# simonmeister/UnFlow

Hardware: NVIDIA H100
Metric: frame-pairs/s at 384x1280 FlowNetC (higher is better)
Workload: dtype f32

## Files before the change

### unflow_b200/csrc/tc_common.cuh

```cuda
#pragma once
#include <cuda.h>

#include "common.cuh"

namespace unflow {
namespace tc {

constexpr int BM = 128;
constexpr int BK = 32;
constexpr int CHUNK = 8;
constexpr int A_BYTES = BM * BK * 4;
extern long long *g_dbg;
extern int g_chunk;

__device__ __forceinline__ unsigned s32(const void *p) { return (unsigned)__cvta_generic_to_shared(p); }

__device__ __forceinline__ void mbar_init(unsigned bar, int count) {
  asm volatile("mbarrier.init.shared::cta.b64 [%0], %1;" ::"r"(bar), "r"(count));
}
__device__ __forceinline__ void mbar_arrive(unsigned bar) {
  asm volatile("mbarrier.arrive.shared::cta.b64 _, [%0];" ::"r"(bar) : "memory");
}
__device__ __forceinline__ void mbar_expect_tx(unsigned bar, unsigned bytes) {
  asm volatile("mbarrier.arrive.expect_tx.shared::cta.b64 _, [%0], %1;" ::"r"(bar), "r"(bytes) : "memory");
}
__device__ __forceinline__ void mbar_wait(unsigned bar, unsigned parity) {
  unsigned done;
  do {
    asm volatile(
        "{\n .reg .pred p;\n mbarrier.try_wait.parity.shared::cta.b64 p, [%1], %2;\n"
        " selp.u32 %0, 1, 0, p;\n}\n"
        : "=r"(done) : "r"(bar), "r"(parity) : "memory");
  } while (!done);
}
__device__ __forceinline__ bool elect_one() {
  unsigned pred = 0;
  asm volatile("{\n .reg .pred p;\n elect.sync _|p, 0xFFFFFFFF;\n selp.u32 %0, 1, 0, p;\n}\n" : "=r"(pred));
  return pred != 0;
}
__device__ __forceinline__ void tma_4d(unsigned dst, const CUtensorMap *map, unsigned bar, int c0, int c1,
                                       int c2, int c3) {
  asm volatile(
      "cp.async.bulk.tensor.4d.shared::cluster.global.tile.mbarrier::complete_tx::bytes"
      " [%0], [%1, {%3, %4, %5, %6}], [%2];"
      ::"r"(dst), "l"(map), "r"(bar), "r"(c0), "r"(c1), "r"(c2), "r"(c3) : "memory");
}
__device__ __forceinline__ void tma_3d(unsigned dst, const CUtensorMap *map, unsigned bar, int c0, int c1,
                                       int c2) {
  asm volatile(
      "cp.async.bulk.tensor.3d.shared::cluster.global.tile.mbarrier::complete_tx::bytes"
      " [%0], [%1, {%3, %4, %5}], [%2];"
      ::"r"(dst), "l"(map), "r"(bar), "r"(c0), "r"(c1), "r"(c2) : "memory");
}
__device__ __forceinline__ void fence_proxy_async() {
  asm volatile("fence.proxy.async.shared::cta;" ::: "memory");
}
__device__ __forceinline__ void named_bar_sync(int id, int count) {
  asm volatile("bar.sync %0, %1;" ::"r"(id), "r"(count) : "memory");
}

__device__ __forceinline__ float tf32_rna(float x) {
  unsigned u;
  asm("cvt.rna.tf32.f32 %0, %1;" : "=r"(u) : "f"(x));
  return __uint_as_float(u);
}
__device__ __forceinline__ float tf32_rna_fast(float x) {
  return __uint_as_float((__float_as_uint(x) + 0x1000u) & 0xFFFFE000u);
}
__device__ __forceinline__ float4 tf32_hi4(float4 v) {
  return make_float4(tf32_rna_fast(v.x), tf32_rna_fast(v.y), tf32_rna_fast(v.z), tf32_rna_fast(v.w));
}
__device__ __forceinline__ float4 sub4(float4 a, float4 b) { return make_float4(a.x - b.x, a.y - b.y, a.z - b.z, a.w - b.w); }

__device__ __forceinline__ void red_add_f32(float *addr, float v) {
  asm volatile("red.global.add.f32 [%0], %1;" ::"l"(addr), "f"(v) : "memory");
}

__device__ __forceinline__ unsigned long long wgmma_desc_k128(unsigned saddr) {
  return (unsigned long long)((saddr >> 4) & 0x3FFFu) | (1ull << 16) | (64ull << 32) | (1ull << 62);
}
__device__ __forceinline__ unsigned sw128_offset(int r, int k) {
  return (unsigned)(r * 128 + ((((k >> 2) ^ (r & 7)) & 7) << 4) + ((k & 3) << 2));
}
__device__ __forceinline__ void wgmma_fence() { asm volatile("wgmma.fence.sync.aligned;" ::: "memory"); }
__device__ __forceinline__ void wgmma_commit() { asm volatile("wgmma.commit_group.sync.aligned;" ::: "memory"); }
template <int N>
__device__ __forceinline__ void wgmma_wait() { asm volatile("wgmma.wait_group.sync.aligned %0;" ::"n"(N) : "memory"); }
template <int R>
__device__ __forceinline__ void fence_regs(float (&d)[R]) {
#pragma unroll
  for (int i = 0; i < R; ++i) asm volatile("" : "+f"(d[i])::"memory");
}
template <int N> struct Wgmma;
template <> struct Wgmma<32> {
  static __device__ __forceinline__ void mma(float (&d)[16], unsigned long long da, unsigned long long db, int scale_d) {
    asm volatile(
        "{\n .reg .pred p;\n setp.ne.b32 p, %18, 0;\n"
        " wgmma.mma_async.sync.aligned.m64n32k8.f32.tf32.tf32 {%0, %1, %2, %3, %4, %5, %6, %7, %8, %9, %10, %11, %12, %13, %14, %15}, %16, %17, p, 1, 1;\n}\n"
        : "+f"(d[0]), "+f"(d[1]), "+f"(d[2]), "+f"(d[3]), "+f"(d[4]), "+f"(d[5]), "+f"(d[6]), "+f"(d[7]), "+f"(d[8]), "+f"(d[9]), "+f"(d[10]), "+f"(d[11]), "+f"(d[12]), "+f"(d[13]), "+f"(d[14]), "+f"(d[15])
        : "l"(da), "l"(db), "r"(scale_d));
  }
};
template <> struct Wgmma<64> {
  static __device__ __forceinline__ void mma(float (&d)[32], unsigned long long da, unsigned long long db, int scale_d) {
    asm volatile(
        "{\n .reg .pred p;\n setp.ne.b32 p, %34, 0;\n"
        " wgmma.mma_async.sync.aligned.m64n64k8.f32.tf32.tf32 {%0, %1, %2, %3, %4, %5, %6, %7, %8, %9, %10, %11, %12, %13, %14, %15, %16, %17, %18, %19, %20, %21, %22, %23, %24, %25, %26, %27, %28, %29, %30, %31}, %32, %33, p, 1, 1;\n}\n"
        : "+f"(d[0]), "+f"(d[1]), "+f"(d[2]), "+f"(d[3]), "+f"(d[4]), "+f"(d[5]), "+f"(d[6]), "+f"(d[7]), "+f"(d[8]), "+f"(d[9]), "+f"(d[10]), "+f"(d[11]), "+f"(d[12]), "+f"(d[13]), "+f"(d[14]), "+f"(d[15]), "+f"(d[16]), "+f"(d[17]), "+f"(d[18]), "+f"(d[19]), "+f"(d[20]), "+f"(d[21]), "+f"(d[22]), "+f"(d[23]), "+f"(d[24]), "+f"(d[25]), "+f"(d[26]), "+f"(d[27]), "+f"(d[28]), "+f"(d[29]), "+f"(d[30]), "+f"(d[31])
        : "l"(da), "l"(db), "r"(scale_d));
  }
};
template <> struct Wgmma<128> {
  static __device__ __forceinline__ void mma(float (&d)[64], unsigned long long da, unsigned long long db, int scale_d) {
    asm volatile(
        "{\n .reg .pred p;\n setp.ne.b32 p, %66, 0;\n"
        " wgmma.mma_async.sync.aligned.m64n128k8.f32.tf32.tf32 {%0, %1, %2, %3, %4, %5, %6, %7, %8, %9, %10, %11, %12, %13, %14, %15, %16, %17, %18, %19, %20, %21, %22, %23, %24, %25, %26, %27, %28, %29, %30, %31, %32, %33, %34, %35, %36, %37, %38, %39, %40, %41, %42, %43, %44, %45, %46, %47, %48, %49, %50, %51, %52, %53, %54, %55, %56, %57, %58, %59, %60, %61, %62, %63}, %64, %65, p, 1, 1;\n}\n"
        : "+f"(d[0]), "+f"(d[1]), "+f"(d[2]), "+f"(d[3]), "+f"(d[4]), "+f"(d[5]), "+f"(d[6]), "+f"(d[7]), "+f"(d[8]), "+f"(d[9]), "+f"(d[10]), "+f"(d[11]), "+f"(d[12]), "+f"(d[13]), "+f"(d[14]), "+f"(d[15]), "+f"(d[16]), "+f"(d[17]), "+f"(d[18]), "+f"(d[19]), "+f"(d[20]), "+f"(d[21]), "+f"(d[22]), "+f"(d[23]), "+f"(d[24]), "+f"(d[25]), "+f"(d[26]), "+f"(d[27]), "+f"(d[28]), "+f"(d[29]), "+f"(d[30]), "+f"(d[31]), "+f"(d[32]), "+f"(d[33]), "+f"(d[34]), "+f"(d[35]), "+f"(d[36]), "+f"(d[37]), "+f"(d[38]), "+f"(d[39]), "+f"(d[40]), "+f"(d[41]), "+f"(d[42]), "+f"(d[43]), "+f"(d[44]), "+f"(d[45]), "+f"(d[46]), "+f"(d[47]), "+f"(d[48]), "+f"(d[49]), "+f"(d[50]), "+f"(d[51]), "+f"(d[52]), "+f"(d[53]), "+f"(d[54]), "+f"(d[55]), "+f"(d[56]), "+f"(d[57]), "+f"(d[58]), "+f"(d[59]), "+f"(d[60]), "+f"(d[61]), "+f"(d[62]), "+f"(d[63])
        : "l"(da), "l"(db), "r"(scale_d));
  }
};

typedef CUresult (*EncodeTiledFn)(CUtensorMap *, CUtensorMapDataType, cuuint32_t, void *, const cuuint64_t *,
                                  const cuuint64_t *, const cuuint32_t *, const cuuint32_t *,
                                  CUtensorMapInterleave, CUtensorMapSwizzle, CUtensorMapL2promotion,
                                  CUtensorMapFloatOOBfill);
inline EncodeTiledFn encode_fn() {
  static EncodeTiledFn fn = nullptr;
  static bool tried = false;
  if (!tried) {
    tried = true;
    void *ptr = nullptr;
    cudaDriverEntryPointQueryResult q;
    if (cudaGetDriverEntryPoint("cuTensorMapEncodeTiled", &ptr, cudaEnableDefault, &q) == cudaSuccess &&
        q == cudaDriverEntryPointSuccess)
      fn = (EncodeTiledFn)ptr;
  }
  return fn;
}
inline int encode(CUtensorMap *m, const float *basep, int rank, const cuuint64_t *dims,
                  const cuuint64_t *strides_bytes, const cuuint32_t *box, const cuuint32_t *estr,
                  CUtensorMapSwizzle swizzle = CU_TENSOR_MAP_SWIZZLE_128B) {
  if (bind_primary_context()) return UNFLOW_ECUDA;
  EncodeTiledFn fn = encode_fn();
  if (!fn) { set_error("cuTensorMapEncodeTiled entry point not available"); return UNFLOW_ECUDA; }
  CUresult r = fn(m, CU_TENSOR_MAP_DATA_TYPE_FLOAT32, (cuuint32_t)rank, (void *)basep, dims, strides_bytes, box,
                  estr, CU_TENSOR_MAP_INTERLEAVE_NONE, swizzle,
                  CU_TENSOR_MAP_L2_PROMOTION_L2_256B, CU_TENSOR_MAP_FLOAT_OOB_FILL_NONE);
  if (r != CUDA_SUCCESS) { set_error("cuTensorMapEncodeTiled failed (%d)", (int)r); return UNFLOW_ECUDA; }
  return UNFLOW_OK;
}

}
}
```

### unflow_b200/csrc/tc_conv.cu

```cuda
#include <algorithm>

#include "tc_common.cuh"

namespace unflow {
namespace tc {

constexpr int MAX_TAPS = 64;
constexpr int NTHREADS = 384;

struct Tap {
  short dx, dy;
  int widx;
  int widx2;
};

struct ConvParams {
  int N, Hit, Wit;
  int TW, TH, TN;
  int tiles_x, tiles_y, tiles_n, n_blocks, n_classes;
  int s_in_x, s_in_y, s_out;
  int Cin, Cout, kblocks;
  float *out;
  long long out_pitch;
  int Hout, Wout;
  const float *bias;
  float slope;
  int act, accumulate;
  int chunk;
  long long *dbg;
  int pair_px;
  int ksplit;
  int class_start[5];
  short class_px[4], class_py[4];
  Tap taps[MAX_TAPS];
};

template <int BN>
struct Cfg {
  static constexpr int B_BYTES = BN * BK * 4;
  static constexpr int STAGE_BYTES = 2 * A_BYTES + 2 * B_BYTES;
  static constexpr int B_OFF = 2 * A_BYTES;
  static constexpr int STAGES = (200 * 1024 / STAGE_BYTES) < 8 ? (200 * 1024 / STAGE_BYTES) : 8;
  static constexpr int SMEM_BYTES = STAGES * STAGE_BYTES + 1024  + 256 ;
  static_assert(STAGES >= 2, "at least two stages");
};

struct TileCoord {
  int cls, n0, iy0, ix0, nb;
};
__device__ __forceinline__ TileCoord decode_tile(const ConvParams &p, int tile) {
  TileCoord t;
  t.nb = tile % p.n_blocks; tile /= p.n_blocks;
  t.cls = tile % p.n_classes; tile /= p.n_classes;
  t.ix0 = (tile % p.tiles_x) * p.TW; tile /= p.tiles_x;
  t.iy0 = (tile % p.tiles_y) * p.TH; tile /= p.tiles_y;
  t.n0 = tile * p.TN;
  return t;
}

struct Work {
  TileCoord t;
  int it0, iters;
};
__device__ __forceinline__ Work decode_work(const ConvParams &p, int w) {
  Work k;
  const int tile = w / p.ksplit, ks = w - tile * p.ksplit;
  k.t = decode_tile(p, tile);
  const int total = (p.class_start[k.t.cls + 1] - p.class_start[k.t.cls]) * p.kblocks;
  const int per = (total + p.ksplit - 1) / p.ksplit;
  k.it0 = ks * per;
  k.iters = total - k.it0 < per ? total - k.it0 : per;
  if (k.iters < 0) k.iters = 0;
  return k;
}

template <int BN>
__global__ void __launch_bounds__(NTHREADS, 1)
tc_conv_kernel(const __grid_constant__ CUtensorMap mapA, const __grid_constant__ CUtensorMap mapBhi,
               const __grid_constant__ CUtensorMap mapBlo, const __grid_constant__ ConvParams p) {
  using C = Cfg<BN>;
  constexpr int R = BN / 2;
  extern __shared__ unsigned char smem_raw[];
  const unsigned base = (s32(smem_raw) + 1023u) & ~1023u;
  unsigned char *gbase = smem_raw + (base - s32(smem_raw));
  const unsigned bars = base + C::STAGES * C::STAGE_BYTES;
  auto full = [&](int s) { return bars + 8u * s; };
  auto empty = [&](int s) { return bars + 8u * (C::STAGES + s); };

  const int warp = __shfl_sync(0xffffffffu, threadIdx.x >> 5, 0), lane = threadIdx.x & 31;
  const int m_tiles = p.tiles_n * p.tiles_y * p.tiles_x;
  const int total_items = p.n_classes * m_tiles * p.n_blocks * p.ksplit;

  if (threadIdx.x == 0) {
    for (int s = 0; s < C::STAGES; ++s) {
      mbar_init(full(s), 1);
      mbar_init(empty(s), 8);
    }
    asm volatile("fence.mbarrier_init.release.cluster;" ::: "memory");
    asm volatile("prefetch.tensormap [%0];" ::"l"(&mapA) : "memory");
    asm volatile("prefetch.tensormap [%0];" ::"l"(&mapBhi) : "memory");
    asm volatile("prefetch.tensormap [%0];" ::"l"(&mapBlo) : "memory");
  }
  __syncthreads();

  if (warp == 0) {
    int s = 0;
    unsigned ph = 0;
    long long t_wait = 0, t_all = clock64();
    const unsigned a_box_bytes = (unsigned)(p.TW * p.TH * p.TN) * BK * 4u;
    for (int item = blockIdx.x; item < total_items; item += gridDim.x) {
      const Work wk = decode_work(p, item);
      const TileCoord t = wk.t;
      const int x0 = p.s_in_x * t.ix0, y0 = p.s_in_y * t.iy0;
      int ti = p.class_start[t.cls] + wk.it0 / p.kblocks, kc = wk.it0 % p.kblocks;
      for (int it = 0; it < wk.iters; ++it) {
        const Tap tap = p.taps[ti];
        { const long long t0 = clock64(); mbar_wait(empty(s), ph ^ 1u); t_wait += clock64() - t0; }
        const unsigned st = base + s * C::STAGE_BYTES;
        if (elect_one()) {
          mbar_expect_tx(full(s), a_box_bytes + 2u * C::B_BYTES);
          tma_4d(st, &mapA, full(s), kc * BK, x0 + tap.dx, y0 + tap.dy, t.n0);
          if (p.pair_px) {
            const int w0 = tap.widx < 0 ? (1 << 20) : tap.widx, w1 = tap.widx2 < 0 ? (1 << 20) : tap.widx2;
            tma_3d(st + C::B_OFF, &mapBhi, full(s), kc * BK, 0, w0);
            tma_3d(st + C::B_OFF + C::B_BYTES / 2, &mapBhi, full(s), kc * BK, 0, w1);
            tma_3d(st + C::B_OFF + C::B_BYTES, &mapBlo, full(s), kc * BK, 0, w0);
            tma_3d(st + C::B_OFF + C::B_BYTES + C::B_BYTES / 2, &mapBlo, full(s), kc * BK, 0, w1);
          } else {
            tma_3d(st + C::B_OFF, &mapBhi, full(s), kc * BK, t.nb * BN, tap.widx);
            tma_3d(st + C::B_OFF + C::B_BYTES, &mapBlo, full(s), kc * BK, t.nb * BN, tap.widx);
          }
        }
        __syncwarp();
        if (++s == C::STAGES) { s = 0; ph ^= 1u; }
        if (++kc == p.kblocks) { kc = 0; ++ti; }
      }
    }
    if (p.dbg && blockIdx.x == 0 && lane == 0) { p.dbg[0] = t_wait; p.dbg[1] = clock64() - t_all; }
  } else if (warp >= 4) {
    const int cw = (warp >> 2) - 1;
    const int ct = threadIdx.x - 128 * (cw + 1);
    const int row0 = 64 * cw + 16 * (ct >> 5) + (lane >> 2);
    const int col0 = 2 * (lane & 3);
    const int per_img = p.TW * p.TH;
    int s = 0;
    unsigned ph = 0;
    long long t_wait = 0, t_all = clock64();
    float sum[R], acc[R];
    for (int item = blockIdx.x; item < total_items; item += gridDim.x) {
      const Work wk = decode_work(p, item);
      const TileCoord t = wk.t;
      const int iters = wk.iters;
#pragma unroll
      for (int c = 0; c < R; ++c) sum[c] = 0.f;
      for (int c0 = 0; c0 < iters; c0 += p.chunk) {
        const int c1 = c0 + p.chunk < iters ? c0 + p.chunk : iters;
        int pending = -1;
        for (int it = c0; it < c1; ++it) {
          { const long long t0 = clock64(); mbar_wait(full(s), ph); t_wait += clock64() - t0; }
          {
            float4 *a = reinterpret_cast<float4 *>(gbase + s * C::STAGE_BYTES + cw * (A_BYTES / 2));
            float4 *l = reinterpret_cast<float4 *>(gbase + s * C::STAGE_BYTES + A_BYTES + cw * (A_BYTES / 2));
#pragma unroll
            for (int j = 0; j < A_BYTES / 2 / 16 / 128; ++j) {
              const int i = ct + 128 * j;
              const float4 v = a[i], h = tf32_hi4(v);
              a[i] = h;
              l[i] = sub4(v, h);
            }
          }
          fence_proxy_async();
          named_bar_sync(1 + cw, 128);
          const unsigned st = base + s * C::STAGE_BYTES;
          const unsigned long long a_hi = wgmma_desc_k128(st + cw * (A_BYTES / 2));
          const unsigned long long a_lo = wgmma_desc_k128(st + A_BYTES + cw * (A_BYTES / 2));
          const unsigned long long b_hi = wgmma_desc_k128(st + C::B_OFF), b_lo = wgmma_desc_k128(st + C::B_OFF + C::B_BYTES);
          fence_regs(acc);
          wgmma_fence();
#pragma unroll
          for (int k = 0; k < BK / 8; ++k) {
            const unsigned long long adv = (unsigned long long)(2 * k);
            Wgmma<BN>::mma(acc, a_lo + adv, b_hi + adv, (it - c0 | k) != 0);
            Wgmma<BN>::mma(acc, a_hi + adv, b_lo + adv, 1);
            Wgmma<BN>::mma(acc, a_hi + adv, b_hi + adv, 1);
          }
          wgmma_commit();
          wgmma_wait<1>();
          fence_regs(acc);
          __syncwarp();
          if (pending >= 0 && lane == 0) mbar_arrive(empty(pending));
          pending = s;
          if (++s == C::STAGES) { s = 0; ph ^= 1u; }
        }
        wgmma_wait<0>();
        fence_regs(acc);
        __syncwarp();
        if (lane == 0) mbar_arrive(empty(pending));
#pragma unroll
        for (int c = 0; c < R; ++c) sum[c] += acc[c];
      }
#pragma unroll
      for (int h = 0; h < 2; ++h) {
        const int row = row0 + 8 * h;
        const int tn = row / per_img, rem = row - tn * per_img;
        const int ty = rem / p.TW, tx = rem - ty * p.TW;
        const int n = t.n0 + tn, iy = t.iy0 + ty, ix = t.ix0 + tx;
        if (!(tn < p.TN && n < p.N && iy < p.Hit && ix < p.Wit)) continue;
        const int oy = p.s_out * iy + p.class_py[t.cls];
        float *const orow = p.out + ((long long)n * p.Hout + oy) * p.Wout * p.out_pitch;
#pragma unroll
        for (int j = 0; j < BN / 8; ++j) {
          const int col = 8 * j + col0;
          const int half = p.pair_px && col >= BN / 2 ? 1 : 0;
          const int c = p.pair_px ? col - half * (BN / 2) : t.nb * BN + col;
          const int ox = p.s_out * ix + (p.pair_px ? half : p.class_px[t.cls]);
          if (c >= p.Cout) continue;
          float *dst = orow + (long long)ox * p.out_pitch + c;
          float v0 = sum[4 * j + 2 * h], v1 = sum[4 * j + 2 * h + 1];
          const bool two = c + 1 < p.Cout;
          if (p.ksplit > 1) {
            if (iters > 0) {
              red_add_f32(dst, v0);
              if (two) red_add_f32(dst + 1, v1);
            }
            continue;
          }
          if (p.bias) {
            v0 += __ldg(p.bias + c);
            if (two) v1 += __ldg(p.bias + c + 1);
          }
          if (p.act) {
            v0 = v0 > 0.f ? v0 : p.slope * v0;
            v1 = v1 > 0.f ? v1 : p.slope * v1;
          }
          if (two) {
            float2 *o = reinterpret_cast<float2 *>(dst);
            if (p.accumulate) { const float2 old = *o; v0 += old.x; v1 += old.y; }
            *o = make_float2(v0, v1);
          } else {
            *dst = p.accumulate ? *dst + v0 : v0;
          }
        }
      }
    }
    if (p.dbg && blockIdx.x == 0 && threadIdx.x == 128) { p.dbg[2] = t_wait; p.dbg[3] = clock64() - t_all; }
  }
}

__global__ void __launch_bounds__(256)
wsplit_kernel(const float *__restrict__ w, float *__restrict__ hi, float *__restrict__ lo, int taps, int R,
              int C, int Cp, long long s_t, long long s_r, long long s_c, int r_fast) {
  __shared__ float tile[32][33];
  const int t = blockIdx.z;
  const int r0 = blockIdx.y * 32, c0 = blockIdx.x * 32;
  const int tx = threadIdx.x & 31, ty = threadIdx.x >> 5;
  for (int k = ty; k < 32; k += 8) {
    const int r = r0 + (r_fast ? tx : k), c = c0 + (r_fast ? k : tx);
    float v = 0.f;
    if (r < R && c < C) v = w[t * s_t + r * s_r + c * s_c];
    if (r_fast) tile[tx][k] = v; else tile[k][tx] = v;
  }
  __syncthreads();
  for (int k = ty; k < 32; k += 8) {
    const int r = r0 + k, c = c0 + tx;
    if (r < R && c < Cp) {
      const float v = tile[k][tx];
      const float h = tf32_rna(v);
      const long long o = ((long long)t * R + r) * Cp + c;
      hi[o] = h;
      lo[o] = v - h;
    }
  }
}

static int floordiv(int a, int b) { return (a >= 0) ? a / b : -((-a + b - 1) / b); }

int g_chunk = CHUNK;
int g_pair_px = 1;
int g_ksplit = 1;
long long *g_dbg = nullptr;

template <int BN>
static int launch(const CUtensorMap &mA, const CUtensorMap &mBh, const CUtensorMap &mBl, const ConvParams &p,
                  cudaStream_t stream) {
  using C = Cfg<BN>;
  static bool attr_set = false;
  if (!attr_set) {
    cudaError_t e = cudaFuncSetAttribute(tc_conv_kernel<BN>, cudaFuncAttributeMaxDynamicSharedMemorySize, C::SMEM_BYTES);
    if (e != cudaSuccess) { set_error("tc_conv: cannot opt in to %d bytes of shared memory: %s", C::SMEM_BYTES, cudaGetErrorString(e)); return UNFLOW_ECUDA; }
    attr_set = true;
  }
  const long long total = (long long)p.n_classes * p.tiles_n * p.tiles_y * p.tiles_x * p.n_blocks * p.ksplit;
  const int grid = total < kNumSMs ? (int)total : kNumSMs;
  tc_conv_kernel<BN><<<grid, NTHREADS, C::SMEM_BYTES, stream>>>(mA, mBh, mBl, p);
  count_launch();
  return check_launch("tc_conv_kernel");
}

inline int choose_ksplit(const ConvParams &p) {
  if (!g_ksplit) return 1;
  const long long items = (long long)p.n_classes * p.tiles_n * p.tiles_y * p.tiles_x * p.n_blocks;
  if (2 * items > kNumSMs) return 1;
  int min_iters = 1 << 30;
  for (int c = 0; c < p.n_classes; ++c) min_iters = std::min(min_iters, (p.class_start[c + 1] - p.class_start[c]) * p.kblocks);
  const long long ks = std::min<long long>(std::min<long long>(kNumSMs / items, 4), std::max(1, min_iters / (4 * p.chunk)));
  return ks < 1 ? 1 : (int)ks;
}

static int launch_bn(int BN, const CUtensorMap &mA, const float *w_hi, const float *w_lo, const cuuint64_t *wdims,
                     const cuuint64_t *wstrides, const ConvParams &p, cudaStream_t stream) {
  CUtensorMap mBh, mBl;
  cuuint32_t box[3] = {(cuuint32_t)BK, (cuuint32_t)(p.pair_px ? BN / 2 : BN), 1};
  cuuint32_t estr[3] = {1, 1, 1};
  int rc = encode(&mBh, w_hi, 3, wdims, wstrides, box, estr);
  if (rc) return rc;
  rc = encode(&mBl, w_lo, 3, wdims, wstrides, box, estr);
  if (rc) return rc;
  if (BN == 128) return launch<128>(mA, mBh, mBl, p, stream);
  if (BN == 64) return launch<64>(mA, mBh, mBl, p, stream);
  return launch<32>(mA, mBh, mBl, p, stream);
}

}
int set_tc_chunk(int v) { if (v < 1 || v > 64) return 0; tc::g_chunk = v; return 1; }
int set_tc_ksplit(int v) { if (v != 0 && v != 1) return 0; tc::g_ksplit = v; return 1; }
int set_tc_pair_px(int v) { if (v != 0 && v != 1) return 0; tc::g_pair_px = v; return 1; }
}

using namespace unflow;

extern "C" int unflow_bias_lrelu(float *y, const float *bias, long long pixels, int C, float slope, void *stream);

extern "C" int unflow_tc_wsplit(const float *w, float *w_hi, float *w_lo, int taps, int R, int C, long long s_t,
                                long long s_r, long long s_c, void *stream) {
  UNFLOW_REQUIRE(w && w_hi && w_lo && taps > 0 && R > 0 && C > 0, "tc_wsplit: bad arguments");
  UNFLOW_REQUIRE(taps <= 65535 && (R + 31) / 32 <= 65535, "tc_wsplit: too many taps / rows");
  const int Cp = (C + 3) / 4 * 4;
  dim3 grid((Cp + 31) / 32, (R + 31) / 32, taps);
  tc::wsplit_kernel<<<grid, 256, 0, (cudaStream_t)stream>>>(w, w_hi, w_lo, taps, R, C, Cp, s_t, s_r, s_c,
                                                           (s_r == 1 && s_c != 1) ? 1 : 0);
  count_launch();
  return check_launch("tc_wsplit_kernel");
}

static int make_plan(tc::ConvParams &p, int &BN, int N, int Hin, int Win, int Cin, int Hout, int Wout, int Cout,
                     int mode, int stride, int kh, int kw, int pad_t, int pad_l) {
  UNFLOW_REQUIRE(N > 0 && Hin > 0 && Win > 0 && Cin > 0 && Hout > 0 && Wout > 0 && Cout > 0, "tc_conv: bad extents");
  UNFLOW_REQUIRE(mode == 0 || mode == 1, "tc_conv: mode must be 0 (conv) or 1 (transposed)");
  UNFLOW_REQUIRE(stride == 1 || stride == 2, "tc_conv: stride must be 1 or 2");
  UNFLOW_REQUIRE(kh > 0 && kw > 0 && kh * kw <= tc::MAX_TAPS, "tc_conv: at most %d taps", tc::MAX_TAPS);
  p.N = N; p.Cin = Cin; p.Cout = Cout; p.kblocks = (Cin + tc::BK - 1) / tc::BK; p.chunk = tc::g_chunk; p.dbg = tc::g_dbg; p.ksplit = 1;
  p.Hout = Hout; p.Wout = Wout;
  int nt = 0;
  if (mode == 0) {
    p.n_classes = 1; p.s_in_x = p.s_in_y = stride; p.s_out = 1; p.Hit = Hout; p.Wit = Wout;
    p.class_px[0] = p.class_py[0] = 0;
    p.class_start[0] = 0;
    for (int ky = 0; ky < kh; ++ky)
      for (int kx = 0; kx < kw; ++kx) p.taps[nt++] = tc::Tap{(short)(kx - pad_l), (short)(ky - pad_t), ky * kw + kx};
    p.class_start[1] = nt;
  } else {
    UNFLOW_REQUIRE(Hout % stride == 0 && Wout % stride == 0, "tc_conv: transposed output extents must be multiples of the stride");
    p.n_classes = stride * stride; p.s_in_x = p.s_in_y = 1; p.s_out = stride; p.Hit = Hout / stride; p.Wit = Wout / stride;
    int c = 0;
    for (int py = 0; py < stride; ++py)
      for (int px = 0; px < stride; ++px, ++c) {
        p.class_px[c] = (short)px; p.class_py[c] = (short)py;
        p.class_start[c] = nt;
        for (int ky = 0; ky < kh; ++ky) {
          if (((py + pad_t - ky) % stride + stride) % stride) continue;
          for (int kx = 0; kx < kw; ++kx) {
            if (((px + pad_l - kx) % stride + stride) % stride) continue;
            UNFLOW_REQUIRE(nt < tc::MAX_TAPS, "tc_conv: too many taps");
            p.taps[nt++] = tc::Tap{(short)tc::floordiv(px + pad_l - kx, stride),
                                   (short)tc::floordiv(py + pad_t - ky, stride), ky * kw + kx};
          }
        }
      }
    p.class_start[p.n_classes] = nt;
    for (int c2 = 0; c2 < p.n_classes; ++c2)
      UNFLOW_REQUIRE(p.class_start[c2 + 1] > p.class_start[c2], "tc_conv: an output parity class has no taps");
  }
  long long best = -1;
  for (int TW = 1; TW <= p.Wit && TW <= 128; ++TW)
    for (int TH = 1; TH <= p.Hit && TW * TH <= 128; ++TH) {
      int TN = 128 / (TW * TH);
      if (TN > N) TN = N;
      const long long tiles = (long long)((p.Wit + TW - 1) / TW) * ((p.Hit + TH - 1) / TH) * ((N + TN - 1) / TN);
      if (best < 0 || tiles < best || (tiles == best && TW > p.TW)) {
        best = tiles; p.TW = TW; p.TH = TH; p.TN = TN;
      }
    }
  p.tiles_x = (p.Wit + p.TW - 1) / p.TW; p.tiles_y = (p.Hit + p.TH - 1) / p.TH; p.tiles_n = (N + p.TN - 1) / p.TN;
  BN = Cout > 64 ? 128 : (Cout > 32 ? 64 : 32);
  p.n_blocks = (Cout + BN - 1) / BN;
  const long long total = (long long)p.n_classes * p.tiles_n * p.tiles_y * p.tiles_x * p.n_blocks;
  UNFLOW_REQUIRE(total < (1ll << 30), "tc_conv: too many tiles");
  return UNFLOW_OK;
// ... 135 lines not shown
```

### unflow_b200/csrc/tc_wgrad.cu

```cuda
#include "tc_common.cuh"

namespace unflow {
namespace tcw {

using namespace unflow::tc;

constexpr int NTHREADS = 384;
constexpr int KP = 32;

struct WgradParams {
  int N, Hp, Wp;
  int TW, TH, TN;
  int tiles_x, tiles_y, tiles_n;
  int n_ptiles, kc, n_chunks;
  int R, C;
  int cgroups, vgroups;
  int r_blocks, c_blocks, taps, kw;
  int chunk;
  long long *dbg;
  int stride, stride_x, pad_t, pad_l;
  float *dw;
  long long pitch_r, pitch_t;
};

constexpr int SMEM_LIMIT = 232448;

template <int BN>
struct Cfg {
  static constexpr int G_BYTES = BN * KP * 4;
  static constexpr int A_HI = 0;
  static constexpr int A_LO = A_HI + A_BYTES;
  static constexpr int B_HI = A_LO + A_BYTES;
  static constexpr int B_LO = B_HI + G_BYTES;
  static constexpr int SPLIT_BYTES = B_LO + G_BYTES;
  static constexpr int SPLIT_STAGES = 2;
  static constexpr int G_RAW = A_BYTES;
  static constexpr int RAW_BYTES = A_BYTES + G_BYTES;
  static constexpr int RAW0 = SPLIT_STAGES * SPLIT_BYTES;
  static constexpr int FIXED = RAW0 + 1024  + 256 ;
  static constexpr int RAW_STAGES = (SMEM_LIMIT - FIXED) / RAW_BYTES < 8 ? (SMEM_LIMIT - FIXED) / RAW_BYTES : 8;
  static constexpr int SMEM_BYTES = FIXED + RAW_STAGES * RAW_BYTES;
  static_assert(RAW_STAGES >= 3, "TMA at least two K blocks ahead of the split");
  static_assert(SMEM_BYTES <= SMEM_LIMIT, "over the shared memory of a block");
  static_assert(8 * (2 * RAW_STAGES + SPLIT_STAGES) <= 256, "barriers");
};

struct Item {
  int chunk, rb, cb;
};
__device__ __forceinline__ Item decode_item(const WgradParams &p, int it) {
  Item w;
  w.cb = it % p.c_blocks; it /= p.c_blocks;
  w.rb = it % p.r_blocks; it /= p.r_blocks;
  w.chunk = it;
  return w;
}
__device__ __forceinline__ int chunk_len(const WgradParams &p, int chunk) {
  const int k0 = chunk * p.kc;
  return (k0 + p.kc <= p.n_ptiles) ? p.kc : p.n_ptiles - k0;
}

template <int ROWS>
__device__ __forceinline__ void split_transpose(const float *raw, unsigned char *hi, unsigned char *lo, int row0, int ct) {
#pragma unroll
  for (int j = 0; j < ROWS * 8 / 128; ++j) {
    const int i = ct + 128 * j;
    const int r = row0 + i % ROWS, c = i / ROWS;
    const float *src = raw + (r >> 5) * 1024 + (4 * c) * 32 + (r & 31);
    const float4 v = make_float4(src[0], src[32], src[64], src[96]), h = tf32_hi4(v);
    const unsigned o = sw128_offset(r, 4 * c);
    *reinterpret_cast<float4 *>(hi + o) = h;
    *reinterpret_cast<float4 *>(lo + o) = sub4(v, h);
  }
}

template <int BN>
__global__ void __launch_bounds__(NTHREADS, 1)
tc_wgrad_kernel(const __grid_constant__ CUtensorMap mapP, const __grid_constant__ CUtensorMap mapG,
                const __grid_constant__ WgradParams p) {
  using C = Cfg<BN>;
  constexpr int R = BN / 2;
  constexpr int GROUPS = BN / 32;
  extern __shared__ unsigned char smem_raw[];
  const unsigned base = (s32(smem_raw) + 1023u) & ~1023u;
  unsigned char *gbase = smem_raw + (base - s32(smem_raw));
  const unsigned bars = base + C::RAW0 + C::RAW_STAGES * C::RAW_BYTES;
  auto raw_full = [&](int s) { return bars + 8u * s; };
  auto raw_empty = [&](int s) { return bars + 8u * (C::RAW_STAGES + s); };
  auto split_empty = [&](int s) { return bars + 8u * (2 * C::RAW_STAGES + s); };

  const int warp = __shfl_sync(0xffffffffu, threadIdx.x >> 5, 0), lane = threadIdx.x & 31;
  const int total_items = p.n_chunks * p.r_blocks * p.c_blocks;

  if (threadIdx.x == 0) {
    for (int s = 0; s < C::RAW_STAGES; ++s) {
      mbar_init(raw_full(s), 1);
      mbar_init(raw_empty(s), 8);
    }
    for (int s = 0; s < C::SPLIT_STAGES; ++s) mbar_init(split_empty(s), 8);
    asm volatile("fence.mbarrier_init.release.cluster;" ::: "memory");
    asm volatile("prefetch.tensormap [%0];" ::"l"(&mapP) : "memory");
    asm volatile("prefetch.tensormap [%0];" ::"l"(&mapG) : "memory");
  }
  __syncthreads();

  if (warp == 0) {
    int s = 0;
    unsigned ph = 0;
    long long t_wait = 0, t_all = clock64();
    for (int item = blockIdx.x; item < total_items; item += gridDim.x) {
      const Item w = decode_item(p, item);
      int gch[GROUPS], gdx[GROUPS], gdy[GROUPS];
#pragma unroll
      for (int j = 0; j < GROUPS; ++j) {
        const int v = w.cb * GROUPS + j;
        if (v < p.vgroups) {
          const int tap = v / p.cgroups, ky = tap / p.kw;
          gch[j] = (v - tap * p.cgroups) * 32; gdy[j] = ky - p.pad_t; gdx[j] = tap - ky * p.kw - p.pad_l;
        } else {
          gch[j] = p.cgroups * 32; gdx[j] = gdy[j] = 0;
        }
      }
      const int k0 = w.chunk * p.kc, klen = chunk_len(p, w.chunk);
      for (int kb = k0; kb < k0 + klen; ++kb) {
        int q = kb;
        const int px = (q % p.tiles_x) * p.TW; q /= p.tiles_x;
        const int py = (q % p.tiles_y) * p.TH; q /= p.tiles_y;
        const int pn = q * p.TN;
        { const long long t0 = clock64(); mbar_wait(raw_empty(s), ph ^ 1u); t_wait += clock64() - t0; }
        const unsigned st = base + C::RAW0 + s * C::RAW_BYTES;
        if (elect_one()) {
          mbar_expect_tx(raw_full(s), (unsigned)C::RAW_BYTES);
#pragma unroll
          for (int j = 0; j < BM / 32; ++j)
            tma_4d(st + j * 4096, &mapP, raw_full(s), w.rb * BM + 32 * j, px, py, pn);
#pragma unroll
          for (int j = 0; j < GROUPS; ++j)
            tma_4d(st + C::G_RAW + j * 4096, &mapG, raw_full(s), gch[j], p.stride_x * px + gdx[j],
                   p.stride * py + gdy[j], pn);
        }
        __syncwarp();
        if (++s == C::RAW_STAGES) { s = 0; ph ^= 1u; }
      }
    }
    if (p.dbg && blockIdx.x == 0 && lane == 0) { p.dbg[0] = t_wait; p.dbg[1] = clock64() - t_all; }
  } else if (warp >= 4) {
    const int cw = (warp >> 2) - 1;
    const int ct = threadIdx.x - 128 * (cw + 1);
    const int row0 = 64 * cw + 16 * (ct >> 5) + (lane >> 2);
    const int col0 = 2 * (lane & 3);
    unsigned n = 0;
    unsigned t_wait = 0, t_split = 0;
    const unsigned t_all = (unsigned)clock();
    auto split = [&](bool rows) {
      const unsigned rs = n % C::RAW_STAGES, rph = (n / C::RAW_STAGES) & 1u;
      const unsigned ss = n % C::SPLIT_STAGES, sph = (n / C::SPLIT_STAGES) & 1u;
      { const unsigned t0 = (unsigned)clock(); mbar_wait(raw_full(rs), rph); t_wait += (unsigned)clock() - t0; }
      { const unsigned t0 = (unsigned)clock(); mbar_wait(split_empty(ss), sph ^ 1u); t_split += (unsigned)clock() - t0; }
      const float *raw = reinterpret_cast<const float *>(gbase + C::RAW0 + rs * C::RAW_BYTES);
      unsigned char *sp = gbase + ss * C::SPLIT_BYTES;
      if (rows) split_transpose<64>(raw, sp + C::A_HI, sp + C::A_LO, 64 * cw, ct);
      split_transpose<BN / 2>(raw + C::G_RAW / 4, sp + C::B_HI, sp + C::B_LO, cw * (BN / 2), ct);
      __syncwarp();
      if (lane == 0) mbar_arrive(raw_empty(rs));
      fence_proxy_async();
      named_bar_sync(1, 256);
    };
    float sum[R], acc[R];
    for (int item = blockIdx.x; item < total_items; item += gridDim.x) {
      const Item w = decode_item(p, item);
      const int iters = chunk_len(p, w.chunk);
      if (w.rb * BM + 64 * cw >= p.R) {
        for (int it = 0; it < iters; ++it) {
          split(false);
          if (lane == 0) mbar_arrive(split_empty(n % C::SPLIT_STAGES));
          ++n;
        }
        continue;
// ... 198 lines not shown
```

Before: 136.2.

## Split A operand into tf32 hi/lo in registers and feed register-sourced WGMMA

The conv kernel no longer rewrites the A tile in shared memory as separate hi/lo tf32 halves, which needed a proxy fence and a named barrier per K block. Each consumer now loads its A fragment from the swizzled stage, splits it into hi/lo registers, and issues register-A WGMMAs. Commits are per k-step with a double-buffered fragment set so the split overlaps the in-flight MMAs. Because the lo copy of A is gone, each stage is smaller, so more stages fit under a raised shared-memory limit. setmaxnreg moves registers from producer warps to consumer warps, at the cost of more shared loads per thread and tighter wgmma_wait ordering.

```diff
diff --git a/unflow_b200/csrc/tc_common.cuh b/unflow_b200/csrc/tc_common.cuh
--- a/unflow_b200/csrc/tc_common.cuh
+++ b/unflow_b200/csrc/tc_common.cuh
@@ -10,6 +10,7 @@
 constexpr int BK = 32;
 constexpr int CHUNK = 8;
 constexpr int A_BYTES = BM * BK * 4;
+constexpr int SMEM_LIMIT = 232448;
 extern long long *g_dbg;
 extern int g_chunk;
 
@@ -55,6 +56,10 @@
 __device__ __forceinline__ void fence_proxy_async() {
   asm volatile("fence.proxy.async.shared::cta;" ::: "memory");
 }
+template <int N>
+__device__ __forceinline__ void setmaxnreg_dec() { asm volatile("setmaxnreg.dec.sync.aligned.u32 %0;" ::"n"(N)); }
+template <int N>
+__device__ __forceinline__ void setmaxnreg_inc() { asm volatile("setmaxnreg.inc.sync.aligned.u32 %0;" ::"n"(N)); }
 __device__ __forceinline__ void named_bar_sync(int id, int count) {
   asm volatile("bar.sync %0, %1;" ::"r"(id), "r"(count) : "memory");
 }
@@ -100,6 +105,13 @@
         : "+f"(d[0]), "+f"(d[1]), "+f"(d[2]), "+f"(d[3]), "+f"(d[4]), "+f"(d[5]), "+f"(d[6]), "+f"(d[7]), "+f"(d[8]), "+f"(d[9]), "+f"(d[10]), "+f"(d[11]), "+f"(d[12]), "+f"(d[13]), "+f"(d[14]), "+f"(d[15])
         : "l"(da), "l"(db), "r"(scale_d));
   }
+  static __device__ __forceinline__ void mma_rs(float (&d)[16], const unsigned (&a)[4], unsigned long long db, int scale_d) {
+    asm volatile(
+        "{\n .reg .pred p;\n setp.ne.b32 p, %21, 0;\n"
+        " wgmma.mma_async.sync.aligned.m64n32k8.f32.tf32.tf32 {%0, %1, %2, %3, %4, %5, %6, %7, %8, %9, %10, %11, %12, %13, %14, %15}, {%16, %17, %18, %19}, %20, p, 1, 1;\n}\n"
+        : "+f"(d[0]), "+f"(d[1]), "+f"(d[2]), "+f"(d[3]), "+f"(d[4]), "+f"(d[5]), "+f"(d[6]), "+f"(d[7]), "+f"(d[8]), "+f"(d[9]), "+f"(d[10]), "+f"(d[11]), "+f"(d[12]), "+f"(d[13]), "+f"(d[14]), "+f"(d[15])
+        : "r"(a[0]), "r"(a[1]), "r"(a[2]), "r"(a[3]), "l"(db), "r"(scale_d));
+  }
 };
 template <> struct Wgmma<64> {
   static __device__ __forceinline__ void mma(float (&d)[32], unsigned long long da, unsigned long long db, int scale_d) {
@@ -109,6 +121,13 @@
         : "+f"(d[0]), "+f"(d[1]), "+f"(d[2]), "+f"(d[3]), "+f"(d[4]), "+f"(d[5]), "+f"(d[6]), "+f"(d[7]), "+f"(d[8]), "+f"(d[9]), "+f"(d[10]), "+f"(d[11]), "+f"(d[12]), "+f"(d[13]), "+f"(d[14]), "+f"(d[15]), "+f"(d[16]), "+f"(d[17]), "+f"(d[18]), "+f"(d[19]), "+f"(d[20]), "+f"(d[21]), "+f"(d[22]), "+f"(d[23]), "+f"(d[24]), "+f"(d[25]), "+f"(d[26]), "+f"(d[27]), "+f"(d[28]), "+f"(d[29]), "+f"(d[30]), "+f"(d[31])
         : "l"(da), "l"(db), "r"(scale_d));
   }
+  static __device__ __forceinline__ void mma_rs(float (&d)[32], const unsigned (&a)[4], unsigned long long db, int scale_d) {
+    asm volatile(
+        "{\n .reg .pred p;\n setp.ne.b32 p, %37, 0;\n"
+        " wgmma.mma_async.sync.aligned.m64n64k8.f32.tf32.tf32 {%0, %1, %2, %3, %4, %5, %6, %7, %8, %9, %10, %11, %12, %13, %14, %15, %16, %17, %18, %19, %20, %21, %22, %23, %24, %25, %26, %27, %28, %29, %30, %31}, {%32, %33, %34, %35}, %36, p, 1, 1;\n}\n"
+        : "+f"(d[0]), "+f"(d[1]), "+f"(d[2]), "+f"(d[3]), "+f"(d[4]), "+f"(d[5]), "+f"(d[6]), "+f"(d[7]), "+f"(d[8]), "+f"(d[9]), "+f"(d[10]), "+f"(d[11]), "+f"(d[12]), "+f"(d[13]), "+f"(d[14]), "+f"(d[15]), "+f"(d[16]), "+f"(d[17]), "+f"(d[18]), "+f"(d[19]), "+f"(d[20]), "+f"(d[21]), "+f"(d[22]), "+f"(d[23]), "+f"(d[24]), "+f"(d[25]), "+f"(d[26]), "+f"(d[27]), "+f"(d[28]), "+f"(d[29]), "+f"(d[30]), "+f"(d[31])
+        : "r"(a[0]), "r"(a[1]), "r"(a[2]), "r"(a[3]), "l"(db), "r"(scale_d));
+  }
 };
 template <> struct Wgmma<128> {
   static __device__ __forceinline__ void mma(float (&d)[64], unsigned long long da, unsigned long long db, int scale_d) {
@@ -117,6 +136,13 @@
         " wgmma.mma_async.sync.aligned.m64n128k8.f32.tf32.tf32 {%0, %1, %2, %3, %4, %5, %6, %7, %8, %9, %10, %11, %12, %13, %14, %15, %16, %17, %18, %19, %20, %21, %22, %23, %24, %25, %26, %27, %28, %29, %30, %31, %32, %33, %34, %35, %36, %37, %38, %39, %40, %41, %42, %43, %44, %45, %46, %47, %48, %49, %50, %51, %52, %53, %54, %55, %56, %57, %58, %59, %60, %61, %62, %63}, %64, %65, p, 1, 1;\n}\n"
         : "+f"(d[0]), "+f"(d[1]), "+f"(d[2]), "+f"(d[3]), "+f"(d[4]), "+f"(d[5]), "+f"(d[6]), "+f"(d[7]), "+f"(d[8]), "+f"(d[9]), "+f"(d[10]), "+f"(d[11]), "+f"(d[12]), "+f"(d[13]), "+f"(d[14]), "+f"(d[15]), "+f"(d[16]), "+f"(d[17]), "+f"(d[18]), "+f"(d[19]), "+f"(d[20]), "+f"(d[21]), "+f"(d[22]), "+f"(d[23]), "+f"(d[24]), "+f"(d[25]), "+f"(d[26]), "+f"(d[27]), "+f"(d[28]), "+f"(d[29]), "+f"(d[30]), "+f"(d[31]), "+f"(d[32]), "+f"(d[33]), "+f"(d[34]), "+f"(d[35]), "+f"(d[36]), "+f"(d[37]), "+f"(d[38]), "+f"(d[39]), "+f"(d[40]), "+f"(d[41]), "+f"(d[42]), "+f"(d[43]), "+f"(d[44]), "+f"(d[45]), "+f"(d[46]), "+f"(d[47]), "+f"(d[48]), "+f"(d[49]), "+f"(d[50]), "+f"(d[51]), "+f"(d[52]), "+f"(d[53]), "+f"(d[54]), "+f"(d[55]), "+f"(d[56]), "+f"(d[57]), "+f"(d[58]), "+f"(d[59]), "+f"(d[60]), "+f"(d[61]), "+f"(d[62]), "+f"(d[63])
         : "l"(da), "l"(db), "r"(scale_d));
+  }
+  static __device__ __forceinline__ void mma_rs(float (&d)[64], const unsigned (&a)[4], unsigned long long db, int scale_d) {
+    asm volatile(
+        "{\n .reg .pred p;\n setp.ne.b32 p, %69, 0;\n"
+        " wgmma.mma_async.sync.aligned.m64n128k8.f32.tf32.tf32 {%0, %1, %2, %3, %4, %5, %6, %7, %8, %9, %10, %11, %12, %13, %14, %15, %16, %17, %18, %19, %20, %21, %22, %23, %24, %25, %26, %27, %28, %29, %30, %31, %32, %33, %34, %35, %36, %37, %38, %39, %40, %41, %42, %43, %44, %45, %46, %47, %48, %49, %50, %51, %52, %53, %54, %55, %56, %57, %58, %59, %60, %61, %62, %63}, {%64, %65, %66, %67}, %68, p, 1, 1;\n}\n"
+        : "+f"(d[0]), "+f"(d[1]), "+f"(d[2]), "+f"(d[3]), "+f"(d[4]), "+f"(d[5]), "+f"(d[6]), "+f"(d[7]), "+f"(d[8]), "+f"(d[9]), "+f"(d[10]), "+f"(d[11]), "+f"(d[12]), "+f"(d[13]), "+f"(d[14]), "+f"(d[15]), "+f"(d[16]), "+f"(d[17]), "+f"(d[18]), "+f"(d[19]), "+f"(d[20]), "+f"(d[21]), "+f"(d[22]), "+f"(d[23]), "+f"(d[24]), "+f"(d[25]), "+f"(d[26]), "+f"(d[27]), "+f"(d[28]), "+f"(d[29]), "+f"(d[30]), "+f"(d[31]), "+f"(d[32]), "+f"(d[33]), "+f"(d[34]), "+f"(d[35]), "+f"(d[36]), "+f"(d[37]), "+f"(d[38]), "+f"(d[39]), "+f"(d[40]), "+f"(d[41]), "+f"(d[42]), "+f"(d[43]), "+f"(d[44]), "+f"(d[45]), "+f"(d[46]), "+f"(d[47]), "+f"(d[48]), "+f"(d[49]), "+f"(d[50]), "+f"(d[51]), "+f"(d[52]), "+f"(d[53]), "+f"(d[54]), "+f"(d[55]), "+f"(d[56]), "+f"(d[57]), "+f"(d[58]), "+f"(d[59]), "+f"(d[60]), "+f"(d[61]), "+f"(d[62]), "+f"(d[63])
+        : "r"(a[0]), "r"(a[1]), "r"(a[2]), "r"(a[3]), "l"(db), "r"(scale_d));
   }
 };
 
diff --git a/unflow_b200/csrc/tc_conv.cu b/unflow_b200/csrc/tc_conv.cu
--- a/unflow_b200/csrc/tc_conv.cu
+++ b/unflow_b200/csrc/tc_conv.cu
@@ -38,12 +38,16 @@
 template <int BN>
 struct Cfg {
   static constexpr int B_BYTES = BN * BK * 4;
-  static constexpr int STAGE_BYTES = 2 * A_BYTES + 2 * B_BYTES;
-  static constexpr int B_OFF = 2 * A_BYTES;
-  static constexpr int STAGES = (200 * 1024 / STAGE_BYTES) < 8 ? (200 * 1024 / STAGE_BYTES) : 8;
-  static constexpr int SMEM_BYTES = STAGES * STAGE_BYTES + 1024  + 256 ;
+  static constexpr int STAGE_BYTES = A_BYTES + 2 * B_BYTES;
+  static constexpr int B_OFF = A_BYTES;
+  static constexpr int FIXED = 1024  + 256 ;
+  static constexpr int STAGES = (SMEM_LIMIT - FIXED) / STAGE_BYTES < 8 ? (SMEM_LIMIT - FIXED) / STAGE_BYTES : 8;
+  static constexpr int SMEM_BYTES = STAGES * STAGE_BYTES + FIXED;
   static_assert(STAGES >= 2, "at least two stages");
+  static_assert(SMEM_BYTES <= SMEM_LIMIT, "over the shared memory of a block");
 };
+constexpr int FRAG_SETS = 2;
+static_assert((BK / 8) % FRAG_SETS == 0 && FRAG_SETS <= BK / 8, "fragment sets per K block");
 
 struct TileCoord {
   int cls, n0, iy0, ix0, nb;
@@ -103,6 +107,7 @@
   }
   __syncthreads();
 
+  if (warp < 4) setmaxnreg_dec<40>();
   if (warp == 0) {
     int s = 0;
     unsigned ph = 0;
@@ -138,6 +143,7 @@
     }
     if (p.dbg && blockIdx.x == 0 && lane == 0) { p.dbg[0] = t_wait; p.dbg[1] = clock64() - t_all; }
   } else if (warp >= 4) {
+    setmaxnreg_inc<232>();
     const int cw = (warp >> 2) - 1;
     const int ct = threadIdx.x - 128 * (cw + 1);
     const int row0 = 64 * cw + 16 * (ct >> 5) + (lane >> 2);
@@ -147,6 +153,7 @@
     unsigned ph = 0;
     long long t_wait = 0, t_all = clock64();
     float sum[R], acc[R];
+    unsigned a_hi[FRAG_SETS][4], a_lo[FRAG_SETS][4];
     for (int item = blockIdx.x; item < total_items; item += gridDim.x) {
       const Work wk = decode_work(p, item);
       const TileCoord t = wk.t;
@@ -158,37 +165,32 @@
         int pending = -1;
         for (int it = c0; it < c1; ++it) {
           { const long long t0 = clock64(); mbar_wait(full(s), ph); t_wait += clock64() - t0; }
-          {
-            float4 *a = reinterpret_cast<float4 *>(gbase + s * C::STAGE_BYTES + cw * (A_BYTES / 2));
-            float4 *l = reinterpret_cast<float4 *>(gbase + s * C::STAGE_BYTES + A_BYTES + cw * (A_BYTES / 2));
-#pragma unroll
-            for (int j = 0; j < A_BYTES / 2 / 16 / 128; ++j) {
-              const int i = ct + 128 * j;
-              const float4 v = a[i], h = tf32_hi4(v);
-              a[i] = h;
-              l[i] = sub4(v, h);
-            }
-          }
-          fence_proxy_async();
-          named_bar_sync(1 + cw, 128);
+          const float *a = reinterpret_cast<const float *>(gbase + s * C::STAGE_BYTES);
           const unsigned st = base + s * C::STAGE_BYTES;
-          const unsigned long long a_hi = wgmma_desc_k128(st + cw * (A_BYTES / 2));
-          const unsigned long long a_lo = wgmma_desc_k128(st + A_BYTES + cw * (A_BYTES / 2));
           const unsigned long long b_hi = wgmma_desc_k128(st + C::B_OFF), b_lo = wgmma_desc_k128(st + C::B_OFF + C::B_BYTES);
-          fence_regs(acc);
-          wgmma_fence();
 #pragma unroll
           for (int k = 0; k < BK / 8; ++k) {
+            unsigned (&hi)[4] = a_hi[k % FRAG_SETS], (&lo)[4] = a_lo[k % FRAG_SETS];
+            wgmma_wait<FRAG_SETS - 1>();
+            fence_regs(acc);
+            if (k == FRAG_SETS - 1) {
+              __syncwarp();
+              if (pending >= 0 && lane == 0) mbar_arrive(empty(pending));
+            }
+#pragma unroll
+            for (int e = 0; e < 4; ++e) {
+              const float x = a[sw128_offset(row0 + 8 * (e & 1), 8 * k + (lane & 3) + 4 * (e >> 1)) / 4];
+              const float h = tf32_rna_fast(x);
+              hi[e] = __float_as_uint(h);
+              lo[e] = __float_as_uint(x - h);
+            }
+            wgmma_fence();
             const unsigned long long adv = (unsigned long long)(2 * k);
-            Wgmma<BN>::mma(acc, a_lo + adv, b_hi + adv, (it - c0 | k) != 0);
-            Wgmma<BN>::mma(acc, a_hi + adv, b_lo + adv, 1);
-            Wgmma<BN>::mma(acc, a_hi + adv, b_hi + adv, 1);
-          }
-          wgmma_commit();
-          wgmma_wait<1>();
-          fence_regs(acc);
-          __syncwarp();
-          if (pending >= 0 && lane == 0) mbar_arrive(empty(pending));
+            Wgmma<BN>::mma_rs(acc, lo, b_hi + adv, (it - c0 | k) != 0);
+            Wgmma<BN>::mma_rs(acc, hi, b_lo + adv, 1);
+            Wgmma<BN>::mma_rs(acc, hi, b_hi + adv, 1);
+            wgmma_commit();
+          }
           pending = s;
           if (++s == C::STAGES) { s = 0; ph ^= 1u; }
         }
@@ -243,7 +245,9 @@
         }
       }
     }
-    if (p.dbg && blockIdx.x == 0 && threadIdx.x == 128) { p.dbg[2] = t_wait; p.dbg[3] = clock64() - t_all; }
+    if (p.dbg && blockIdx.x == 0 && threadIdx.x == 128) {
+      p.dbg[2] = t_wait; p.dbg[3] = clock64() - t_all; p.dbg[5] = C::STAGES;
+    }
   }
 }
 
diff --git a/unflow_b200/csrc/tc_wgrad.cu b/unflow_b200/csrc/tc_wgrad.cu
--- a/unflow_b200/csrc/tc_wgrad.cu
+++ b/unflow_b200/csrc/tc_wgrad.cu
@@ -22,8 +22,6 @@
   float *dw;
   long long pitch_r, pitch_t;
 };
-
-constexpr int SMEM_LIMIT = 232448;
 
 template <int BN>
 struct Cfg {
```

New measurement: 142.3, median of 6. 1.04x the previous value.
